# sakehl/SKA-SDP-Accelerate-gridding

Hardware: AMD Instinct MI355X
Metric: Mvis/s gridded (w-proj, 4096^2 grid) (higher is better)
Workload: dtype f64

## Files before the change

ska-sdp-accelerate-gridding_amd/csrc/api.hip:

```cpp

#include "common.h"
#include "imaging.h"

using namespace gridhip;

namespace {

int check_common(gridhip_ctx *ctx, int64_t H, int64_t Wd, const void *grid, int64_t n, const void *u,
                 const void *v, int64_t uv_stride)
{
    if (!ctx) return GRIDHIP_EINVAL;
    if (H <= 0 || Wd <= 0 || n < 0 || uv_stride < 1)
        return fail(ctx, GRIDHIP_EINVAL, "bad size (H=%lld Wd=%lld n=%lld uv_stride=%lld)", (long long)H,
                    (long long)Wd, (long long)n, (long long)uv_stride);
    if (!grid || (n > 0 && (!u || !v))) return fail(ctx, GRIDHIP_EINVAL, "null pointer");
    if (n > (int64_t)0x7fffff00) return fail(ctx, GRIDHIP_EUNSUPPORTED, "n must be < 2^31 per call");
    return GRIDHIP_OK;
}

int check_errors(gridhip_ctx *ctx)
{
    int32_t e = 0;
    GH_CHECK_HIP(ctx, hipMemcpyAsync(&e, ctx->d_scalars + 2, sizeof e, hipMemcpyDeviceToHost, ctx->stream));
    GH_CHECK_HIP(ctx, hipStreamSynchronize(ctx->stream));
// ... 22 lines not shown

static bool choose_parts(int64_t gh, int64_t gw, int side, int *py, int *px, int *sub)
{
    const int y = (int)((gh + side - 1) / side), x = (int)((gw + side - 1) / side);
    const int sy = (int)((gh + y - 1) / y), sx = (int)((gw + x - 1) / x);
    int sb = sy > sx ? sy : sx;
    if (sb < 5) sb = 5;
    if (y * x > 64) return false;
    *py = y;
    *px = x;
    *sub = sb;
    return true;
}

static void sorted_block(gridhip_ctx *ctx, Prep *p)
{
    if (ctx->opt.block != 0) return;
    const size_t per_cu = (size_t)ctx->max_lds / p->lds_sorted;
    p->block = per_cu >= 4 ? 256 : per_cu >= 2 ? 512 : 1024;
}

int prepare(gridhip_ctx *ctx, int64_t H, int64_t Wd, int64_t W, int64_t Q, int64_t gh, int64_t gw, int64_t n, Prep *p)
{
    *p = Prep();
    p->nrec = n;
    int rc = make_geom(ctx, H, Wd, W, Q, gh, gw, n, &p->g, &p->block, &p->lds);
    if (rc == GRIDHIP_OK) {
        const bool want = ctx->opt.sort == 1 || (ctx->opt.sort == 0 && n / (int64_t)p->g.nbins >= 256);
        const bool old_parts = ctx->opt.subfoot == 1 && gh > 16;
        p->sorted = want && !old_parts && sorted_plan(ctx, p->g, p->block, &p->nkeys, &p->batch, &p->lds_sorted);
        if (p->sorted) {
            p->g.chunk = p->batch;
            sorted_block(ctx, p);
        }
        if (p->sorted || ctx->opt.sort == 2) return GRIDHIP_OK;
    } else if (rc != GRIDHIP_EUNSUPPORTED || ctx->opt.tile != 0)
        return rc;
    int py, px, sub;
    const int side = ctx->opt.subfoot == 1 ? 16 : 32;
    if (ctx->opt.sort != 2 && (gh != gw || gh > side || gh < 5) && choose_parts(gh, gw, side, &py, &px, &sub) &&
        n * (int64_t)(py * px) < (int64_t)0x7fffff00 && W * Q * Q * (int64_t)(py * px) < ((int64_t)1 << 30)) {
        Prep q;
        const int P = py * px;
        q.nrec = n * P;
        if (make_geom(ctx, H, Wd, W, Q, sub, sub, q.nrec, &q.g, &q.block, &q.lds, P) == GRIDHIP_OK) {
            q.g.fgh = (int32_t)gh;
            q.g.fgw = (int32_t)gw;
            q.g.py = py;
            q.g.px = px;
            q.g.P = P;
            q.g.nvis = (int32_t)(n > 0 ? n : 1);
            q.g.nslices = (int32_t)(W * Q * Q * P);
            set_rec_bits(&q.g);
            set_div_magic(&q.g);
            const bool want = ctx->opt.sort == 1 || (ctx->opt.sort == 0 && q.nrec / (int64_t)q.g.nbins >= 256);
            q.sorted = want && sorted_plan(ctx, q.g, q.block, &q.nkeys, &q.batch, &q.lds_sorted);
            if (q.sorted) {
                q.g.chunk = q.batch;
                sorted_block(ctx, &q);
                *p = q;
                return GRIDHIP_OK;
            }
        }
    }
    if (rc == GRIDHIP_EUNSUPPORTED) {
        p->direct = true;
        return GRIDHIP_OK;
    }
    return rc;
}

int tile_kernels(gridhip_ctx *ctx, const Prep &p, const double *gcf, const double **out)
{
    ctx->last_path = p.direct ? 4 : !p.sorted ? 3 : p.g.P > 1 || p.g.fgh != p.g.gh || p.g.fgw != p.g.gw ? 2 : 1;
    ctx->last_geom[0] = p.g.ngroups;
    ctx->last_geom[1] = p.g.Tx;
    ctx->last_geom[2] = p.g.Ty;
    ctx->last_geom[3] = p.g.imoff > 0;
    *out = gcf;
    if (p.g.P == 1 && p.g.fgh == p.g.gh && p.g.fgw == p.g.gw) return GRIDHIP_OK;
    const int64_t nsl = (int64_t)p.g.W * p.g.Q * p.g.Q;
    const size_t elems = (size_t)nsl * p.g.P * p.g.gh * p.g.gw;
    GH_CHECK(ws_reserve(ctx, ctx->ktab, elems * 16));
    int blocks = (int)((elems + 255) / 256);
    if (blocks > ctx->num_cu * 16) blocks = ctx->num_cu * 16;
    hipLaunchKernelGGL(pad_kernels_kernel, dim3(blocks), dim3(256), 0, ctx->stream, p.g, nsl, (const double2 *)gcf,
                       (double2 *)ctx->ktab.ptr);
    GH_CHECK_HIP(ctx, hipGetLastError());
    *out = (const double *)ctx->ktab.ptr;
    return GRIDHIP_OK;
}

int upload_inputs(gridhip_ctx *ctx, GridInputs &d, size_t cells, const double *grid, int64_t n, int64_t uv_stride,
                  const double *u, const double *v, const double *vis, const int64_t *wbin, const double *gcf,
                  size_t gcf_elems)
{
    if (grid) {
        GH_CHECK(d.grid.upload(ctx, grid, cells * 16));
    } else {
        GH_CHECK(d.grid.alloc(ctx, cells * 16));
        GH_CHECK_HIP(ctx, hipMemsetAsync(d.grid.p, 0, cells * 16, ctx->stream));
    }
    const size_t span = n > 0 ? (size_t)(n - 1) * uv_stride + 1 : 0;
    GH_CHECK(d.u.upload(ctx, u, span * 8));
    GH_CHECK(d.v.upload(ctx, v, span * 8));
    GH_CHECK(vis ? d.vis.upload(ctx, vis, (size_t)n * 16) : d.vis.alloc(ctx, (size_t)n * 16));
    if (wbin) GH_CHECK(d.wbin.upload(ctx, wbin, (size_t)n * 8));
    if (gcf) GH_CHECK(d.gcf.upload(ctx, gcf, gcf_elems * 16));
    return GRIDHIP_OK;
}

// ... 179 lines not shown
```

ska-sdp-accelerate-gridding_amd/csrc/common.h:

```cpp
#pragma once
#include <hip/hip_runtime.h>
#include <stdint.h>
#include <stdio.h>
#include <string>
#include <unordered_set>

#include "../../include/gridhip.h"

namespace gridhip {

struct VisRec {
    int32_t lxy;
    int32_t kslice;
    int32_t orig;
};
typedef unsigned long long RecWord;

struct Geom {
    int64_t H, Wd;
    int32_t W, Q, gh, gw;
    int32_t Tx, Ty;
    int32_t offx, offy;
    int32_t ntx, nty;
    int32_t ntiles;
    int32_t ngroups;
    int32_t nbins;
    int32_t ldw;
    int32_t lrows, lcols;
    int32_t chunk;
    int32_t dbg;
    int32_t per_vis;
    int32_t nrec;
    int32_t nvis;
    int32_t nslices;
    int32_t fgh, fgw, px, py, P;
    int32_t ob, kb;
    int32_t dense;
    int32_t npersist;
    int32_t budget;
    int32_t imoff;
    uint32_t mTx, mTy, mW, mP, mPx;
    int32_t sTx, sTy, sW, sP, sPx;
};

static inline void div_magic(int64_t d, uint32_t *m, int32_t *s)
{
    if (d <= 1) {
        *m = 0;
        *s = -1;
        return;
    }
    int l = 0;
    while (((int64_t)1 << l) < d) ++l;
    const unsigned __int128 num = (unsigned __int128)1 << (31 + l);
    *m = (uint32_t)((num + (unsigned __int128)d - 1) / (unsigned __int128)d);
    *s = l - 1;
}
__device__ __forceinline__ uint32_t udiv_magic(uint32_t x, uint32_t m, int32_t s)
{
    return s < 0 ? x : __umulhi(x, m) >> s;
}
static inline void set_div_magic(Geom *g)
{
    div_magic(g->Tx, &g->mTx, &g->sTx);
    div_magic(g->Ty, &g->mTy, &g->sTy);
    div_magic(g->W, &g->mW, &g->sW);
    div_magic(g->P, &g->mP, &g->sP);
    div_magic(g->px, &g->mPx, &g->sPx);
}

static inline int bits_for(int64_t count)
{
    int b = 1;
    while (((int64_t)1 << b) < count) ++b;
    return b;
}
// ... 182 lines not shown
```

ska-sdp-accelerate-gridding_amd/csrc/ctx.hip:

```cpp
#include <stdarg.h>
#include <string.h>

#include <stdlib.h>

#include "common.h"
#include "imaging.h"

namespace gridhip {

int fail(gridhip_ctx *ctx, int code, const char *fmt, ...)
{
    char buf[512];
    va_list ap;
    va_start(ap, fmt);
    vsnprintf(buf, sizeof buf, fmt, ap);
    va_end(ap);
    if (ctx) ctx->err = buf;
    return code;
}

int ws_reserve(gridhip_ctx *ctx, Workspace &ws, size_t bytes)
{
    if (bytes <= ws.bytes) return GRIDHIP_OK;
    GH_CHECK_HIP(ctx, hipDeviceSynchronize());
// ... 52 lines not shown
    return l;
}

static int lds_pitch(int lcols, int gw)
{
    int p = lcols;
    while (p % 32 != gw % 32) ++p;
    return p;
}

size_t tables_bytes(const Geom &g)
{
    size_t ints = (size_t)g.nbins + ((size_t)g.nbins + 1) +
                  (size_t)g.ngroups * ((size_t)g.ntiles + 1) + (size_t)g.nbins;
    return ints * sizeof(int32_t);
}

Tables tables_of(gridhip_ctx *ctx, const Geom &g)
{
    Tables t;
    int32_t *p = (int32_t *)ctx->tables.ptr;
    t.bin_count = p;
    p += g.nbins;
    t.bin_start = p;
    p += g.nbins + 1;
    t.work_start = p;
    p += (size_t)g.ngroups * (g.ntiles + 1);
    t.cursor = p;
    t.scalars = ctx->d_scalars;
    return t;
}

static int make_geom1(gridhip_ctx *ctx, int64_t H, int64_t Wd, int64_t W, int64_t Q, int64_t gh, int64_t gw, int64_t n,
                      Geom *g, int *block, size_t *lds_bytes, int parts);

int make_geom(gridhip_ctx *ctx, int64_t H, int64_t Wd, int64_t W, int64_t Q, int64_t gh,
              int64_t gw, int64_t n, Geom *g, int *block, size_t *lds_bytes, int parts)
{
    GH_CHECK(make_geom1(ctx, H, Wd, W, Q, gh, gw, n, g, block, lds_bytes, parts));
    if (g->imoff > 0) {
        const int64_t planes = (W + g->ngroups - 1) / g->ngroups + 1;
        const size_t hist = (size_t)((planes * Q * Q * parts + 1 + 3) & ~(int64_t)3) * 4;
        if (2 * (size_t)g->imoff + hist + 128 > (size_t)ctx->max_lds) GH_CHECK(make_geom1(ctx, H, Wd, W, Q, gh, gw, n, g, block, lds_bytes, 0));
    }
    return GRIDHIP_OK;
}

static int make_geom1(gridhip_ctx *ctx, int64_t H, int64_t Wd, int64_t W, int64_t Q, int64_t gh, int64_t gw, int64_t n,
                      Geom *g, int *block, size_t *lds_bytes, int parts)
{
    if (H <= 0 || Wd <= 0 || W <= 0 || Q <= 0 || gh <= 0 || gw <= 0)
        return fail(ctx, GRIDHIP_EINVAL, "non-positive dimension");
    if (H > (1 << 30) || Wd > (1 << 30) || W * Q * Q > (1LL << 30) || gh > 1024 || gw > 1024)
        return fail(ctx, GRIDHIP_EUNSUPPORTED, "shape outside tile-kernel limits");
    memset(g, 0, sizeof *g);
    g->H = H;
    g->Wd = Wd;
    g->W = (int32_t)W;
    g->Q = (int32_t)Q;
    g->gh = (int32_t)gh;
    g->gw = (int32_t)gw;
    g->nvis = (int32_t)(n > 0 ? n : 1);
    g->nrec = g->nvis;
    g->nslices = (int32_t)(W * Q * Q);
    g->fgh = (int32_t)gh;
    g->fgw = (int32_t)gw;
    g->px = g->py = g->P = 1;
    g->per_vis = 0;
    set_rec_bits(g);
    if (ctx->opt.rec_bits >= 100 && ctx->opt.rec_bits <= 164 && g->ob + g->kb + 14 < ctx->opt.rec_bits - 100)
        g->kb = (int32_t)(ctx->opt.rec_bits - 100) - 14 - g->ob;

    const size_t lds_cap = (size_t)ctx->max_lds - 1024;
    const bool bt_ok = parts > 0 && ctx->opt.bigtile != 2 && ctx->opt.tile == 0 && ctx->opt.tile_x == 0 && gh == gw && gh >= 5 && gh <= 32;
    auto plane_for = [&](int tx, int ty) {
        return (size_t)lds_pitch(tx + (int)gw - 1, (int)gw) * (size_t)(ty + (int)gh - 1) * 8;
    };
    auto tiles_of = [&](int tx, int ty) {
        const int ox = (((int)gw - 1 + tx - 1) / tx) * tx, oy = (((int)gh - 1 + ty - 1) / ty) * ty;
        return (int64_t)((Wd - 1 + ox) / tx + 1) * (int64_t)((H - 1 + oy) / ty + 1);
    };
    auto auto_groups = [&](int64_t ntiles) {
        const double work = (double)n / (double)ntiles * ((double)gh * (double)gw / 225.0);
        return W < 8 ? 1 : work >= 8000.0 ? 8 : work >= 1200.0 ? 4 : work >= 600.0 ? 2 : 1;
    };
    int64_t ng_est = ctx->opt.wgroups ? ctx->opt.wgroups : (W >= 8 ? 8 : 1);
    auto largest_tile = [&](bool big, int *otx, int *oty) {
        const size_t hist_need = (size_t)(((W + ng_est - 1) / ng_est + 2) * Q * Q * (parts > 0 ? parts : 1)) * 4 + 1024;
        const size_t hist_room = big ? hist_need : (hist_need > 24576 && hist_need < 65536 * 4 ? hist_need : 24576);
        const size_t plane_cap = big ? lds_cap : 65528;
        size_t best = 0;
        if (hist_room + 8192 > lds_cap) return best;
        for (int tx = 8; tx <= 128; ++tx) {
            const int pitch = lds_pitch(tx + (int)gw - 1, (int)gw);
            if (tx < 128 && lds_pitch(tx + 1 + (int)gw - 1, (int)gw) == pitch) continue;
            int rows = (int)(plane_cap / ((size_t)pitch * 8));
            if ((size_t)rows * pitch * 16 > lds_cap - hist_room) rows = (int)((lds_cap - hist_room) / ((size_t)pitch * 16));
            int ty = rows - ((int)gh - 1);
            if (ty > 128) ty = 128;
            if (ty < 8) continue;
            if ((size_t)tx * ty > best) {
                best = (size_t)tx * ty;
                *otx = tx;
                *oty = ty;
            }
        }
        return best;
    };
    bool bigtile = false;
    int Tx = (int)ctx->opt.tile_x, Ty = (int)ctx->opt.tile_y;
    if (ctx->opt.tile) Tx = Ty = (int)ctx->opt.tile;
    if ((Tx == 0) != (Ty == 0)) return fail(ctx, GRIDHIP_EINVAL, "tile_x and tile_y go together");
    if (Tx == 0) {
        size_t best = largest_tile(false, &Tx, &Ty);
        if (best > 0 && bt_ok) {
            const int64_t tiles = ((H + Ty - 1) / Ty) * ((Wd + Tx - 1) / Tx);
            const bool sparse = n >= ((int64_t)1 << 22) && n < 2 * tiles * W * Q * Q;
            int bx = 0, by = 0;
            if (!ctx->opt.wgroups) ng_est = auto_groups(tiles_of(Tx, Ty));
            if ((ctx->opt.bigtile == 1 || sparse) && largest_tile(true, &bx, &by) > best) {
                best = (size_t)bx * by;
                Tx = bx;
                Ty = by;
                bigtile = true;
            }
        }
        if (best == 0) {
            Tx = Ty = 8;
            if (plane_for(8, 8) * 2 > lds_cap)
                return fail(ctx, GRIDHIP_EUNSUPPORTED, "a %lldx%lld kernel does not fit an LDS tile", (long long)gh, (long long)gw);
        }
        while ((Tx > 16 || Ty > 16) && ((H + Ty - 1) / Ty) * ((Wd + Tx - 1) / Tx) < 1024) {
            if (Ty >= Tx)
                --Ty;
            else
                --Tx;
        }
    }
    if (Tx < 8 || Tx > 128 || Ty < 8 || Ty > 128) return fail(ctx, GRIDHIP_EINVAL, "tile sides must be in 8..128");
    if (plane_for(Tx, Ty) * 2 > lds_cap)
        return fail(ctx, GRIDHIP_EUNSUPPORTED, "tile %dx%d with %lldx%lld kernel needs %zu B of LDS", Tx, Ty,
                    (long long)gh, (long long)gw, plane_for(Tx, Ty) * 2);
    g->Tx = Tx;
    g->Ty = Ty;
    g->imoff = bigtile && plane_for(Tx, Ty) > 65528 ? (int32_t)plane_for(Tx, Ty) : 0;
    g->lcols = Tx + (int)gw - 1;
    g->lrows = Ty + (int)gh - 1;
    g->ldw = lds_pitch(g->lcols, (int)gw);
    g->offx = (((int)gw - 1 + Tx - 1) / Tx) * Tx;
    g->offy = (((int)gh - 1 + Ty - 1) / Ty) * Ty;
    g->ntx = (int)((Wd - 1 + g->offx) / Tx) + 1;
    g->nty = (int)((H - 1 + g->offy) / Ty) + 1;
    if ((int64_t)g->ntx * g->nty > (1 << 24)) return fail(ctx, GRIDHIP_EUNSUPPORTED, "too many tiles");
    g->ntiles = g->ntx * g->nty;

    int ng = (int)ctx->opt.wgroups;
    if (ng == 0) {
        ng = auto_groups(g->ntiles);
        const int64_t cap = ((int64_t)ctx->max_lds - 8192) / 4;
        if (ng == 8 && (int64_t)g->ntiles * 8 > 4 * cap) ng = 4;
    }
    if (ng > W) ng = (int)W;
    if (W * ng >= ((int64_t)1 << 31)) ng = 1;
    if (ng < 1 || ng > 16) return fail(ctx, GRIDHIP_EINVAL, "wgroups must be in 1..16");
    g->ngroups = ng;
    g->nbins = ng * g->ntiles;
    set_div_magic(g);
    g->dense = ctx->opt.wtable ? (ctx->opt.wtable >= 3 ? 2 : ctx->opt.wtable == 2 ? 1 : 0)
                               : (gh >= 15 && n >= 2 * (int64_t)g->ntiles * W * Q * Q) ? 1 : (g->imoff > 0 && gh == 15) ? 2 : 0;

    int chunk = (int)ctx->opt.chunk;
    if (chunk == 0) chunk = 8192;
    if (chunk < 64) chunk = 64;
    g->chunk = chunk;
    g->dbg = (int32_t)ctx->opt.dbg;

    *lds_bytes = plane_for(Tx, Ty) * 2;
    int b = (int)ctx->opt.block;
    if (b == 0) {
        size_t per_cu = (size_t)ctx->max_lds / *lds_bytes;
        b = per_cu >= 4 ? 256 : per_cu >= 2 ? 512 : 1024;
    }
    if (b < 64 || b > 1024 || (b & 63)) return fail(ctx, GRIDHIP_EINVAL, "block must be a multiple of 64 in 64..1024");
    *block = b;
    (void)n;
    return GRIDHIP_OK;
}

}

using namespace gridhip;

extern "C" {

int gridhip_version(void) { return GRIDHIP_VERSION; }

const char *gridhip_strerror(int code)
{
    switch (code) {
        case GRIDHIP_OK: return "ok";
        case GRIDHIP_EINVAL: return "invalid argument";
        case GRIDHIP_ENOMEM: return "out of memory";
// ... 326 lines not shown
```

ska-sdp-accelerate-gridding_amd/csrc/tile_sorted.hip:

```cpp
#include "tile_common.h"

namespace gridhip {

__device__ __forceinline__ double readlane_f64(double x, int l)
{
    return __hiloint2double(__builtin_amdgcn_readlane(__double2hiint(x), l),
                            __builtin_amdgcn_readlane(__double2loint(x), l));
}

constexpr int SORTED_IM_OFF = 65528;

__device__ const int cut15[3][16] = {{0, 106, 211, 317, 422, 500, 578, 655, 733, 781, 829, 877, 926, 958, 991, 1024},
                                     {0, 108, 221, 329, 434, 513, 596, 677, 754, 800, 852, 898, 943, 969, 998, 1024},
                                     {0, 100, 202, 303, 401, 480, 562, 641, 718, 769, 824, 875, 925, 957, 992, 1024}};

struct SortedItem {
    int32_t valid, tile, grp, staged;
};

template <int S, bool DEGRID, int ABL = 0, bool AW = false, bool BT = false>
__global__ void __launch_bounds__(1024, 4) tile_grid_sorted_kernel(Geom g, const RecWord *__restrict__ recs,
                                                                const int32_t *__restrict__ bin_start,
                                                                const int32_t *__restrict__ work_start,
                                                                const double2 *__restrict__ gcf,
                                                                double2 *__restrict__ vis,
                                                                double *__restrict__ grid, int nkeys, int batch,
                                                                int32_t *__restrict__ scalars,
                                                                double2 *__restrict__ sorted_vals,
                                                                uint2 *__restrict__ sorted_mo)
{
    extern __shared__ double lds[];
    constexpr int S2 = S * S;
    constexpr int TAIL0 = S2 - ((S2 + 63) / 64 - 1) * 64;
    constexpr int EXTRA = DEGRID ? 0 : (TAIL0 > 32 && TAIL0 <= 34) ? TAIL0 - 32 : (S2 > 256 && TAIL0 <= 2) ? TAIL0 : 0;
    constexpr int S2E = S2 - EXTRA;
    constexpr int NSTEP_ALL = (S2E + 63) / 64;
    constexpr int TAIL = S2E - (NSTEP_ALL - 1) * 64;
    constexpr int MAXST = DEGRID ? 4 : 5;
    constexpr int FP = (NSTEP_ALL + MAXST - 1) / MAXST;
    constexpr int KST = (NSTEP_ALL + FP - 1) / FP;
    constexpr int REM = NSTEP_ALL % FP;
    constexpr int PBASE = NSTEP_ALL / FP;
    constexpr int NSTEP = KST;
    constexpr int LASTS = (REM == 0 ? KST : KST - 1) - 1;
    constexpr bool PAIR = !DEGRID && TAIL == 32;
    const int tid = threadIdx.x, nthr = blockDim.x;
    const int lane = tid & 63, wave = __builtin_amdgcn_readfirstlane(tid >> 6), nw = nthr >> 6;
    const int plane = g.lrows * g.ldw;
    const int IMO = BT ? g.imoff / 8 : SORTED_IM_OFF / 8;
    double *lre = lds, *lim = lds + IMO;
    int32_t *hist = reinterpret_cast<int32_t *>(lim + plane);
    const int hist_words = (nkeys + 1 + 3) & ~3;
    SortedItem *desc = reinterpret_cast<SortedItem *>(hist + hist_words);
    double2 *svals_wg = sorted_vals + (size_t)blockIdx.x * 2 * batch;
    uint2 *smo_wg = sorted_mo + (size_t)blockIdx.x * 2 * batch;
    int32_t *sorig_wg = reinterpret_cast<int32_t *>(sorted_vals) + (size_t)blockIdx.x * 2 * batch;

    constexpr bool STAGE_VALS = !DEGRID && AW;
    constexpr bool STAGE_ORIG = DEGRID && AW;
    const bool solo = nw == 1;
    const bool is_sorter = wave == nw - 1;
    if (is_sorter && !solo && !(g.dbg & 512)) __builtin_amdgcn_s_setprio(3);
    const bool is_walker = solo || !is_sorter;
    const int nwalk = solo ? 1 : nw - 1;
    const int ncell = g.lrows * g.lcols;

    if (blockIdx.x == 0 && tid == 0) {
        long long *st = reinterpret_cast<long long *>(scalars + 20);
        st[0] = (long long)__builtin_amdgcn_s_memtime();
        st[1] = (long long)__builtin_amdgcn_s_memrealtime();
    }
    long long prof[7] = {0, 0, 0, 0, 0, 0, 0}, pt = 0;
#define GH_STAMP(i_)                        \
    if ((ABL & 16) && lane == 0) {          \
        const long long now_ = clock64();   \
        prof[i_] += now_ - pt;              \
        pt = now_;                          \
    }
    if ((ABL & 16) && lane == 0) pt = clock64();

    int32_t *queue = scalars + 4;
    int turn = 0;
    int items_left = ((int)blockIdx.x >= g.npersist) ? g.budget : 0x7fffffff;
    auto prepare = [&](int slot) {
// ... 57 lines not shown
            }
            int base = incl - sum;
            for (int i = lo; i < hi; ++i) {
                const int c = hist[i];
                hist[i] = base;
                base += c;
            }
        }
        __builtin_amdgcn_fence(__ATOMIC_ACQ_REL, "wavefront");
        __builtin_amdgcn_wave_barrier();
        GH_STAMP(2)
        int bad = 0;
        for (int r0 = lane; r0 < cnt; r0 += 8 * 64) {
            VisRec rec[8];
            double2 val[8];
            bool off[8];
#pragma unroll
            for (int q = 0; q < 8; ++q) rec[q] = load_rec(recs, b_lo + min(r0 + q * 64, cnt - 1), g, &off[q]);
            if (STAGE_VALS) {
#pragma unroll
                for (int q = 0; q < 8; ++q) val[q] = (ABL & 8) ? make_double2(1.0, (double)q) : load_nt(vis + rec[q].orig);
            }
#pragma unroll
            for (int q = 0; q < 8; ++q) {
                if (r0 + q * 64 >= cnt) break;
                int key = rec[q].kslice - first_slice;
                if (AW) key = (int)((unsigned)key % (unsigned)nkeys);
                if (off[q] || (unsigned)key >= (unsigned)nkeys) {
                    ++bad;
                    continue;
                }
                const int pos = atomicAdd(&hist[key], 1);
                if ((unsigned)pos < (unsigned)batch) {
                    smo[pos] = make_uint2(((uint32_t)key << 16) | (uint32_t)((rec[q].lxy >> 16) * g.ldw + (rec[q].lxy & 0xffff)),
                                          (uint32_t)(AW ? rec[q].kslice : rec[q].orig));
                    if (STAGE_VALS) svals[pos] = val[q];
                    if (STAGE_ORIG) sorig[pos] = rec[q].orig;
                } else
                    ++bad;
            }
        }
        if (bad) atomicAdd(&scalars[2], bad);
        __builtin_amdgcn_fence(__ATOMIC_ACQ_REL, "wavefront");
        __builtin_amdgcn_wave_barrier();
        if (lane == 0) {
            SortedItem d;
            d.valid = 1;
            d.tile = w.tile;
            d.grp = grp;
            d.staged = hist[nkeys - 1];
            desc[slot] = d;
        }
        GH_STAMP(3)
    };

    int loff[NSTEP];
    const bool tail_ok = lane < TAIL || TAIL == 64;
#pragma unroll
    for (int s = 0; s < NSTEP; ++s) {
        int t = s * 64 + lane;
        if (FP == 1 && s == NSTEP - 1 && !tail_ok) t = PAIR ? s * 64 + lane - 32 : 0;
        loff[s] = (t / S) * g.ldw + (t % S);
    }
    const int ttail = tail_ok ? LASTS * 64 + lane : PAIR ? LASTS * 64 + lane - 32 : 0;
    const int lrow = lane / S, lcol = lane - lrow * S;

    auto walk = [&](int slot, int staged, int first_slice) {
        const double2 *svals = svals_wg + (size_t)slot * batch;
        const uint2 *smo = smo_wg + (size_t)slot * batch;
        const int32_t *sorig = sorig_wg + (size_t)slot * batch;
        int seg_lo, seg_hi;
        if (nwalk == 15 && !DEGRID && !(g.dbg & 256)) {
            seg_lo = (int)(((int64_t)staged * cut15[g.dense][wave]) >> 10);
            seg_hi = (int)(((int64_t)staged * cut15[g.dense][wave + 1]) >> 10);
        } else {
            seg_lo = (int)(((int64_t)staged * wave) / nwalk);
            seg_hi = (int)(((int64_t)staged * (wave + 1)) / nwalk);
        }
        if (seg_lo >= seg_hi) return;
        auto load_list = [&](int b0, uint2 &mo, double2 &v, int32_t &o) {
            const int idx = max(min(b0 + lane, seg_hi - 1), seg_lo);
            mo = smo[idx];
            if (STAGE_VALS) v = svals[idx];
            if (STAGE_ORIG) o = sorig[idx];
        };
        auto load_value = [&](const uint2 &mo, double2 &v) {
            if (!DEGRID && !STAGE_VALS) v = (ABL & 8) ? make_double2(1.0, 2.0) : load_nt(vis + mo.y);
        };
        auto part_step0 = [&](int part) { return FP == 1 ? 0 : part * PBASE + min(part, REM); };
        auto part_nst = [&](int part) { return (FP == 1 || REM == 0 || part < REM) ? KST : KST - 1; };
        auto issue = [&](double2(&k)[NSTEP], int key, int len, int part) {
            key = min(max(key, 0), (AW ? g.nslices : nkeys) - 1);
            asm volatile("" : "+s"(key));
            const double2 *kp = gcf + (size_t)(first_slice + key) * S2 + 64 * part_step0(part);
            if (ABL & 4) {
// ... 62 lines not shown
                    return;
                }
                start = (int)__builtin_ctzll(bits);
                bits &= bits - 1;
                len = (bits ? (int)__builtin_ctzll(bits) : bcnt) - start;
                key = lastKey = AW ? __builtin_amdgcn_readlane((int)mo.y, start)
                                   : (int)((uint32_t)__builtin_amdgcn_readlane((int)mo.x, start) >> 16);
                if (FP > 1) {
                    part = 0;
                    curKey = key;
                    curStart = start;
                    curLen = len;
                    curPart = 0;
                }
            };
            auto process = [&](const double2(&k)[NSTEP], int start, int len, int part) {
                int lo[NSTEP];
                const bool lastp = FP == 1 || part == FP - 1;
                const bool shortp = FP > 1 && part_nst(part) < KST;
                if (FP == 1) {
#pragma unroll
                    for (int s = 0; s < NSTEP; ++s) lo[s] = loff[s];
                } else {
                    const int st0 = part_step0(part);
#pragma unroll
                    for (int s = 0; s < NSTEP; ++s) {
                        const int tl = 64 * (st0 + s);
                        const int A = tl / S, B = tl - A * S;
                        int lr = lrow, lc = lcol;
                        if (PAIR && s == LASTS && lastp && lane >= 32) {
                            lr = (lane - 32) / S;
                            lc = (lane - 32) - lr * S;
                        }
                        const int carry = (B + lc >= S) ? g.ldw - S : 0;
                        lo[s] = (A + lr) * g.ldw + B + lc + carry;
                    }
                }
                if (!DEGRID) {
                    int i = 0;
                    if (PAIR && lastp) {
                        for (; i + 1 < len; i += 2) {
                            const int j0 = start + i, j1 = j0 + 1;
                            const int lb0 = (int)((uint32_t)__builtin_amdgcn_readlane((int)mo.x, j0) & 0xffff);
                            const int lb1 = (int)((uint32_t)__builtin_amdgcn_readlane((int)mo.x, j1) & 0xffff);
                            const double vx0 = readlane_f64(vB.x, j0), vy0 = readlane_f64(vB.y, j0);
                            const double vx1 = readlane_f64(vB.x, j1), vy1 = readlane_f64(vB.y, j1);
#pragma unroll
                            for (int s = 0; s < LASTS; ++s) {
                                double *cell = lre + (lb0 + lo[s]);
                                if (ABL & 1) continue;
                                __hip_atomic_fetch_add(cell, vx0 * k[s].x - vy0 * k[s].y, __ATOMIC_RELAXED,
                                                       __HIP_MEMORY_SCOPE_WORKGROUP);
                                __hip_atomic_fetch_add(cell + IMO, vx0 * k[s].y + vy0 * k[s].x,
                                                       __ATOMIC_RELAXED, __HIP_MEMORY_SCOPE_WORKGROUP);
                            }
#pragma unroll
                            for (int s = 0; s < LASTS; ++s) {
                                double *cell = lre + (lb1 + lo[s]);
                                if (ABL & 1) continue;
                                __hip_atomic_fetch_add(cell, vx1 * k[s].x - vy1 * k[s].y, __ATOMIC_RELAXED,
                                                       __HIP_MEMORY_SCOPE_WORKGROUP);
                                __hip_atomic_fetch_add(cell + IMO, vx1 * k[s].y + vy1 * k[s].x,
                                                       __ATOMIC_RELAXED, __HIP_MEMORY_SCOPE_WORKGROUP);
                            }
                            const double2 kl = k[LASTS];
                            double re, im;
                            int a;
                            if (lane < 32) {
// ... 91 lines not shown
            constexpr int NSETS = 3;
            double2 kS[NSETS][NSTEP];
            int keyS[NSETS], startS[NSETS], lenS[NSETS], partS[NSETS] = {0, 0, 0};
            static_assert(NSETS == 3, "initialiser of partS");
#pragma unroll
            for (int r = 0; r < NSETS - 1; ++r) {
                advance(keyS[r], startS[r], lenS[r], partS[r]);
                issue(kS[r], keyS[r], lenS[r], partS[r]);
            }
            int done = 0;
            for (;;) {
#pragma unroll
                for (int r = 0; r < NSETS; ++r) {
                    const int nx = (r + NSETS - 1) % NSETS;
                    advance(keyS[nx], startS[nx], lenS[nx], partS[nx]);
                    issue(kS[nx], keyS[nx], lenS[nx], partS[nx]);
                    asm volatile("" ::: "memory");
                    __builtin_amdgcn_sched_barrier(0);
                    process(kS[r], startS[r], lenS[r], partS[r]);
                    __builtin_amdgcn_sched_barrier(0);
                    if (FP == 1 || partS[r] == FP - 1) done += lenS[r];
                }
                if (done >= bcnt) break;
            }
            if (done > bcnt) {
#pragma unroll
                for (int r = 0; r < NSETS - 1; ++r) asm volatile("" ::"v"(kS[r][0].x), "v"(kS[r][NSTEP - 1].y));
            }
            if (EXTRA > 0 && !(ABL & 1) && lane < bcnt) {
                const int lb = (int)(mo.x & 0xffff);
#pragma unroll
                for (int e = 0; e < EXTRA; ++e) {
                    const int t = S2 - EXTRA + e;
                    double *cell = lre + (lb + (t / S) * g.ldw + (t % S));
                    __hip_atomic_fetch_add(cell, vB.x * kx[e].x - vB.y * kx[e].y, __ATOMIC_RELAXED,
                                           __HIP_MEMORY_SCOPE_WORKGROUP);
                    __hip_atomic_fetch_add(cell + IMO, vB.x * kx[e].y + vB.y * kx[e].x, __ATOMIC_RELAXED,
                                           __HIP_MEMORY_SCOPE_WORKGROUP);
                }
            }
        }
    };

    const int fl_r0 = (tid >> 1) / g.lcols, fl_c0 = (tid >> 1) - fl_r0 * g.lcols;
    const int fl_dr = (nthr >> 1) / g.lcols, fl_dc = (nthr >> 1) - fl_dr * g.lcols;

    if (is_sorter) prepare(0);
    if (!DEGRID) {
        for (int i = tid; i < plane; i += nthr) {
            lre[i] = 0.0;
            lim[i] = 0.0;
        }
    }
    __syncthreads();
    for (int cur = 0;; cur ^= 1) {
        const SortedItem d = desc[cur];
        if (!d.valid) break;
        const int first_plane = (d.grp * g.W + g.ngroups - 1) / g.ngroups;
        const int first_slice = first_plane * g.Q * g.Q * g.P;
        const int tx = d.tile % g.ntx, ty = d.tile / g.ntx;
        const int64_t ox = (int64_t)tx * g.Tx - g.offx, oy = (int64_t)ty * g.Ty - g.offy;
        if (DEGRID) {
            const double2 *gsrc = reinterpret_cast<const double2 *>(grid);
            for (int c = tid; c < ncell; c += nthr) {
                const int r_ = c / g.lcols, c_ = c - r_ * g.lcols;
                const int64_t gx = ox + c_, gy = oy + r_;
                double2 v = make_double2(0.0, 0.0);
                if (gx >= 0 && gy >= 0 && gx < g.Wd && gy < g.H) v = gsrc[gy * g.Wd + gx];
                lre[r_ * g.ldw + c_] = v.x;
                lim[r_ * g.ldw + c_] = v.y;
            }
            __syncthreads();
        }
        const long long walk_t0 = (ABL & 16) ? clock64() : 0;
        if (is_sorter && !solo) prepare(cur ^ 1);
        if (is_walker) {
            if ((ABL & 16) && wave == 0 && lane == 0) pt = clock64();
            walk(cur, d.staged, first_slice);
            if ((ABL & 16) && wave == 0) GH_STAMP(4)
        }
        if (solo) prepare(cur ^ 1);
        if ((ABL & 16) && lane == 0)
            atomicAdd(reinterpret_cast<unsigned long long *>(scalars + 32) + 8 + wave, (unsigned long long)(clock64() - walk_t0));
        __syncthreads();
        if ((ABL & 16) && wave == 0) GH_STAMP(5)
        if (DEGRID) continue;

        {
            const int comp = tid & 1;
            int r_ = fl_r0, c_ = fl_c0;
            for (int e = tid; e < 2 * ncell; e += nthr) {
                const int64_t gx = ox + c_, gy = oy + r_;
                double *cell = (comp ? lim : lre) + r_ * g.ldw + c_;
                c_ += fl_dc;
                r_ += fl_dr;
                if (c_ >= g.lcols) {
                    c_ -= g.lcols;
                    ++r_;
                }
                const double val = *cell;
                if (val == 0.0) continue;
                *cell = 0.0;
                if ((ABL & 2) || gx < 0 || gy < 0 || gx >= g.Wd || gy >= g.H) continue;
                unsafeAtomicAdd(grid + 2 * (gy * g.Wd + gx) + comp, val);
            }
        }
        __syncthreads();
        if ((ABL & 16) && wave == 0) GH_STAMP(6)
    }
    if (blockIdx.x == 0 && tid == 0) {
        long long *st = reinterpret_cast<long long *>(scalars + 20);
        st[2] = (long long)__builtin_amdgcn_s_memtime();
        st[3] = (long long)__builtin_amdgcn_s_memrealtime();
    }
    if ((ABL & 16) && lane == 0 && (wave == 0 || (is_sorter && !solo))) {
        unsigned long long *out = reinterpret_cast<unsigned long long *>(scalars + 32);
        for (int i = 0; i < 7; ++i)
            if (prof[i]) atomicAdd(&out[i], (unsigned long long)prof[i]);
    }
#undef GH_STAMP
}

bool sorted_plan(const gridhip_ctx *ctx, const Geom &g, int block, int *nkeys, int *batch, size_t *lds_bytes)
{
    if (g.gh != g.gw || g.gh < 5 || g.gh > (g.per_vis ? 16 : 32)) return false;
    const int planes = (g.W + g.ngroups - 1) / g.ngroups + 1;
    const int64_t keys = g.per_vis ? 4096 : (int64_t)planes * g.Q * g.Q * g.P;
    if (keys >= 65536) return false;
    const size_t plane = (size_t)g.lrows * g.ldw * 8;
    if (plane > (size_t)(g.imoff > 0 ? g.imoff : SORTED_IM_OFF)) return false;
    const size_t tile = (size_t)(g.imoff > 0 ? g.imoff : SORTED_IM_OFF) + plane;
    const size_t hist = (size_t)((keys + 1 + 3) & ~3) * 4;
    if (tile + hist + 128 > (size_t)ctx->max_lds) return false;
    (void)block;
    int c = ctx->opt.chunk ? (int)ctx->opt.chunk : 16384;
    c = c < 64 ? 64 : c > 16384 ? 16384 : c;
    *nkeys = (int)keys;
    *batch = c;
    *lds_bytes = tile + hist + 128;
    return true;
}

int launch_tile_grid_sorted(gridhip_ctx *ctx, const Geom &g_in, int block, size_t lds_bytes, int nkeys, int batch,
                            int64_t n, const double *gcf, const double *vis, double *grid, bool degrid)
{
    Geom g = g_in;
    Tables t = tables_of(ctx, g);
    const RecWord *recs = (const RecWord *)ctx->recs.ptr;
    if (g.chunk > batch) return fail(ctx, GRIDHIP_EINVAL, "sorted kernel: chunk %d exceeds its work-item capacity %d", g.chunk, batch);
    if (g.per_vis && g.imoff > 0) return fail(ctx, GRIDHIP_EUNSUPPORTED, "no big-tile form of the aw tile kernel");
    int per_cu = (int)((size_t)ctx->max_lds / lds_bytes);
    per_cu = per_cu < 1 ? 1 : per_cu > 4 ? 4 : per_cu;
    if (per_cu * block > 2048) per_cu = 2048 / block > 0 ? 2048 / block : 1;
    int cus = ctx->num_cu - (int)ctx->opt.reserve_cus;
    if (cus < g.ngroups) cus = g.ngroups;
    int nblk = cus * per_cu;
    nblk = ctx->opt.reserve_cus ? (nblk / g.ngroups) * g.ngroups : ((nblk + g.ngroups - 1) / g.ngroups) * g.ngroups;
    const int most = work_blocks(g, n);
    if (nblk > most) nblk = most > g.ngroups ? (most / g.ngroups) * g.ngroups : g.ngroups;
    g.npersist = nblk;
    g.budget = 0;
    if (ctx->opt.yield_cus > 0 && !ctx->opt.reserve_cus) {
        int k = (((int)ctx->opt.yield_cus + 31) / 32) * 32 * per_cu;
        k = (k / g.ngroups) * g.ngroups;
        if (k > 0 && nblk - k >= g.ngroups) {
            g.npersist = nblk - k;
            g.budget = 8;
            int extra = most - g.npersist;
            extra = extra > 2048 ? 2048 : extra;
            extra = (extra / g.ngroups) * g.ngroups;
            nblk = g.npersist + (extra > k ? extra : k);
        }
    }
    const dim3 gr(nblk), bl(block);
    const size_t nlist = (size_t)nblk * 2 * batch, nvals = g.per_vis ? nlist : 0;
    GH_CHECK(ws_reserve(ctx, ctx->sorted, nvals * 16 + nlist * 8));
    double2 *svals = (double2 *)ctx->sorted.ptr;
    uint2 *smo = (uint2 *)(svals + nvals);
    launch_clear(ctx, t.scalars + 4, 16, (g.dbg & 16) ? t.scalars + 32 : nullptr, (g.dbg & 16) ? 64 : 0);
#define GH_LAUNCH_(S_, D_, B_)                                                                                   \
    do {                                                                                                         \
        GH_CHECK(raise_lds(ctx, tile_grid_sorted_kernel<S_, D_, 0, false, B_>));                                 \
        hipLaunchKernelGGL((tile_grid_sorted_kernel<S_, D_, 0, false, B_>), gr, bl, lds_bytes, ctx->stream, g, recs, \
                           t.bin_start, t.work_start, (const double2 *)gcf, (double2 *)vis, grid, nkeys, batch, \
                           t.scalars, svals, smo);                                                               \
    } while (0)
#define GH_LAUNCH(S_, D_)                \
    do {                                 \
        if (g.imoff > 0)                 \
            GH_LAUNCH_(S_, D_, true);    \
        else                             \
            GH_LAUNCH_(S_, D_, false);   \
    } while (0)
#define GH_LAUNCH_AW_(S_, D_)                                                                                    \
    do {                                                                                                         \
        GH_CHECK(raise_lds(ctx, tile_grid_sorted_kernel<S_, D_, 0, true>));                                      \
        hipLaunchKernelGGL((tile_grid_sorted_kernel<S_, D_, 0, true>), gr, bl, lds_bytes, ctx->stream, g, recs,  \
                           t.bin_start, t.work_start, (const double2 *)gcf, (double2 *)vis, grid, nkeys, batch, \
                           t.scalars, svals, smo);                                                               \
    } while (0)
#define GH_LAUNCH_AW(S_)                 \
    do {                                 \
        if (degrid)                      \
            GH_LAUNCH_AW_(S_, true);     \
        else                             \
            GH_LAUNCH_AW_(S_, false);    \
    } while (0)
#define GH_CASE(S_)             \
    case S_:                    \
        if (g.per_vis)          \
            GH_LAUNCH_AW(S_);   \
        else if (degrid)        \
            GH_LAUNCH(S_, true); \
        else                    \
            GH_LAUNCH(S_, false); \
        break;
#define GH_BIG(S_)                                                                  \
    case S_:                                                                        \
        if (g.per_vis) return fail(ctx, GRIDHIP_EUNSUPPORTED, "aw tile kernel: support %d", g.gh); \
        if (degrid)                                                                 \
            GH_LAUNCH(S_, true);                                                    \
        else                                                                        \
            GH_LAUNCH(S_, false);                                                   \
        break;
#define GH_ABL_BT(A_)                                                                                            \
    if (g.gh == 15 && !degrid && g.imoff > 0 && g.dbg == A_) {                                                   \
        GH_CHECK(raise_lds(ctx, tile_grid_sorted_kernel<15, false, A_, false, true>));                           \
        hipLaunchKernelGGL((tile_grid_sorted_kernel<15, false, A_, false, true>), gr, bl, lds_bytes, ctx->stream, g, recs, \
                           t.bin_start, t.work_start, (const double2 *)gcf, (double2 *)vis, grid, nkeys, batch, \
                           t.scalars, svals, smo);                                                               \
        GH_CHECK_HIP(ctx, hipGetLastError());                                                                    \
        return GRIDHIP_OK;                                                                                       \
    }
#define GH_ABL(A_)                                                                                               \
    if (g.gh == 15 && !degrid && g.imoff == 0 && g.dbg == A_) {                                                  \
        GH_CHECK(raise_lds(ctx, tile_grid_sorted_kernel<15, false, A_>));                                        \
        hipLaunchKernelGGL((tile_grid_sorted_kernel<15, false, A_>), gr, bl, lds_bytes, ctx->stream, g, recs,    \
                           t.bin_start, t.work_start, (const double2 *)gcf, (double2 *)vis, grid, nkeys, batch, \
                           t.scalars, svals, smo);                                                               \
        GH_CHECK_HIP(ctx, hipGetLastError());                                                                    \
        return GRIDHIP_OK;                                                                                       \
    }
#ifdef GRIDHIP_TUNING
    GH_ABL(1) GH_ABL(2) GH_ABL(3) GH_ABL(4) GH_ABL(5) GH_ABL(7) GH_ABL(8) GH_ABL(15) GH_ABL(16) GH_ABL_BT(16)
#endif
#undef GH_ABL
#undef GH_ABL_BT
    switch (g.gh) {
        GH_CASE(5) GH_CASE(6) GH_CASE(7) GH_CASE(8) GH_CASE(9) GH_CASE(10) GH_CASE(11) GH_CASE(12) GH_CASE(13)
        GH_CASE(14) GH_CASE(15) GH_CASE(16)
        GH_BIG(17) GH_BIG(18) GH_BIG(19) GH_BIG(20) GH_BIG(21) GH_BIG(22) GH_BIG(23) GH_BIG(24) GH_BIG(25) GH_BIG(26)
        GH_BIG(27) GH_BIG(28) GH_BIG(29) GH_BIG(30) GH_BIG(31) GH_BIG(32)
        default: return fail(ctx, GRIDHIP_EUNSUPPORTED, "no sorted instantiation for support %d", g.gh);
    }
#undef GH_CASE
#undef GH_BIG
#undef GH_LAUNCH
#undef GH_LAUNCH_
#undef GH_LAUNCH_AW
#undef GH_LAUNCH_AW_
    GH_CHECK_HIP(ctx, hipGetLastError());
    return GRIDHIP_OK;
}

}
```

Before: 9171.

## Interleave real/imag LDS planes with a compile-time offset and tuned row pitch

Replaces the sorted tile kernel's split real/imag LDS layout, which used a fixed 64 KB imaginary-plane offset or a runtime big-tile offset, with a per-support compile-time distance between real and imaginary cells inside a shared row of pitch R. The row pitch is chosen to keep bank alignment and to maximise the tile area that fits in LDS. This is meant to fit larger tiles into LDS without a separate BT template variant and to make the imaginary offset a constant, which reduces halo overhead and address arithmetic. It adds new geometry constraints and fallbacks when the layout does not fit, and it changes how tiles are sized on the non-big path.

```diff
diff --git a/ska-sdp-accelerate-gridding_amd/csrc/api.hip b/ska-sdp-accelerate-gridding_amd/csrc/api.hip
--- a/ska-sdp-accelerate-gridding_amd/csrc/api.hip
+++ b/ska-sdp-accelerate-gridding_amd/csrc/api.hip
@@ -78,6 +78,10 @@
         if (p->sorted) {
             p->g.chunk = p->batch;
             sorted_block(ctx, p);
+        }
+        if (!p->sorted && p->g.big) {
+            rc = make_geom(ctx, H, Wd, W, Q, gh, gw, n, &p->g, &p->block, &p->lds, -1);
+            if (rc != GRIDHIP_OK) return rc;
         }
         if (p->sorted || ctx->opt.sort == 2) return GRIDHIP_OK;
     } else if (rc != GRIDHIP_EUNSUPPORTED || ctx->opt.tile != 0)
@@ -122,7 +126,7 @@
     ctx->last_geom[0] = p.g.ngroups;
     ctx->last_geom[1] = p.g.Tx;
     ctx->last_geom[2] = p.g.Ty;
-    ctx->last_geom[3] = p.g.imoff > 0;
+    ctx->last_geom[3] = p.g.big;
     *out = gcf;
     if (p.g.P == 1 && p.g.fgh == p.g.gh && p.g.fgw == p.g.gw) return GRIDHIP_OK;
     const int64_t nsl = (int64_t)p.g.W * p.g.Q * p.g.Q;
diff --git a/ska-sdp-accelerate-gridding_amd/csrc/common.h b/ska-sdp-accelerate-gridding_amd/csrc/common.h
--- a/ska-sdp-accelerate-gridding_amd/csrc/common.h
+++ b/ska-sdp-accelerate-gridding_amd/csrc/common.h
@@ -38,10 +38,34 @@
     int32_t dense;
     int32_t npersist;
     int32_t budget;
-    int32_t imoff;
+    int32_t sR, sD, big;
     uint32_t mTx, mTy, mW, mP, mPx;
     int32_t sTx, sTy, sW, sP, sPx;
 };
+
+constexpr int SORTED_LDS_CELLS = (160 * 1024 - 1024 - 5632) / 8;
+constexpr int sorted_pitch(int cols, int S)
+{
+    int p = cols;
+    while (p % 32 != S % 32) ++p;
+    return p;
+}
+constexpr int sorted_im_dist(int S)
+{
+    int best = 0, dist = 0;
+    for (int pass = 0; pass < 2; ++pass)
+        for (int R = sorted_pitch(2 * (8 + S - 1), S); R <= 2 * (128 + S - 1) + 32; R += 32) {
+            int lcols = R / 2;
+            if (lcols > 128 + S - 1) lcols = 128 + S - 1;
+            int ty = SORTED_LDS_CELLS / R - (S - 1);
+            if (ty > 128) ty = 128;
+            if (ty < 8) continue;
+            const int cells = (lcols - (S - 1)) * ty;
+            if (pass == 0 && cells > best) best = cells;
+            if (pass == 1 && dist == 0 && cells * 100 >= best * 99) dist = R - lcols;
+        }
+    return dist;
+}
 
 static inline void div_magic(int64_t d, uint32_t *m, int32_t *s)
 {
diff --git a/ska-sdp-accelerate-gridding_amd/csrc/ctx.hip b/ska-sdp-accelerate-gridding_amd/csrc/ctx.hip
--- a/ska-sdp-accelerate-gridding_amd/csrc/ctx.hip
+++ b/ska-sdp-accelerate-gridding_amd/csrc/ctx.hip
@@ -108,22 +108,22 @@
 }
 
 static int make_geom1(gridhip_ctx *ctx, int64_t H, int64_t Wd, int64_t W, int64_t Q, int64_t gh, int64_t gw, int64_t n,
-                      Geom *g, int *block, size_t *lds_bytes, int parts);
+                      Geom *g, int *block, size_t *lds_bytes, int parts, bool allow_big);
 
 int make_geom(gridhip_ctx *ctx, int64_t H, int64_t Wd, int64_t W, int64_t Q, int64_t gh,
               int64_t gw, int64_t n, Geom *g, int *block, size_t *lds_bytes, int parts)
 {
-    GH_CHECK(make_geom1(ctx, H, Wd, W, Q, gh, gw, n, g, block, lds_bytes, parts));
-    if (g->imoff > 0) {
+    GH_CHECK(make_geom1(ctx, H, Wd, W, Q, gh, gw, n, g, block, lds_bytes, parts, true));
+    if (g->big) {
         const int64_t planes = (W + g->ngroups - 1) / g->ngroups + 1;
         const size_t hist = (size_t)((planes * Q * Q * parts + 1 + 3) & ~(int64_t)3) * 4;
-        if (2 * (size_t)g->imoff + hist + 128 > (size_t)ctx->max_lds) GH_CHECK(make_geom1(ctx, H, Wd, W, Q, gh, gw, n, g, block, lds_bytes, 0));
+        if ((size_t)g->sR * g->lrows * 8 + hist + 128 > (size_t)ctx->max_lds) GH_CHECK(make_geom1(ctx, H, Wd, W, Q, gh, gw, n, g, block, lds_bytes, parts, false));
     }
     return GRIDHIP_OK;
 }
 
 static int make_geom1(gridhip_ctx *ctx, int64_t H, int64_t Wd, int64_t W, int64_t Q, int64_t gh, int64_t gw, int64_t n,
-                      Geom *g, int *block, size_t *lds_bytes, int parts)
+                      Geom *g, int *block, size_t *lds_bytes, int parts, bool allow_big)
 {
     if (H <= 0 || Wd <= 0 || W <= 0 || Q <= 0 || gh <= 0 || gw <= 0)
         return fail(ctx, GRIDHIP_EINVAL, "non-positive dimension");
@@ -148,7 +148,7 @@
         g->kb = (int32_t)(ctx->opt.rec_bits - 100) - 14 - g->ob;
 
     const size_t lds_cap = (size_t)ctx->max_lds - 1024;
-    const bool bt_ok = parts > 0 && ctx->opt.bigtile != 2 && ctx->opt.tile == 0 && ctx->opt.tile_x == 0 && gh == gw && gh >= 5 && gh <= 32;
+    const bool bt_ok = allow_big && parts > 0 && ctx->opt.bigtile != 2 && ctx->opt.tile == 0 && ctx->opt.tile_x == 0 && gh == gw && gh >= 5 && gh <= 32;
     auto plane_for = [&](int tx, int ty) {
         return (size_t)lds_pitch(tx + (int)gw - 1, (int)gw) * (size_t)(ty + (int)gh - 1) * 8;
     };
@@ -161,17 +161,36 @@
         return W < 8 ? 1 : work >= 8000.0 ? 8 : work >= 1200.0 ? 4 : work >= 600.0 ? 2 : 1;
     };
     int64_t ng_est = ctx->opt.wgroups ? ctx->opt.wgroups : (W >= 8 ? 8 : 1);
+    const int sD = gh == gw && gh >= 5 && gh <= 32 ? sorted_im_dist((int)gh) : 0;
+    auto sorted_row = [&](int lcols) { return sD > 0 && lcols <= sD ? sorted_pitch(sD + lcols, (int)gw) : 0; };
     auto largest_tile = [&](bool big, int *otx, int *oty) {
         const size_t hist_need = (size_t)(((W + ng_est - 1) / ng_est + 2) * Q * Q * (parts > 0 ? parts : 1)) * 4 + 1024;
         const size_t hist_room = big ? hist_need : (hist_need > 24576 && hist_need < 65536 * 4 ? hist_need : 24576);
-        const size_t plane_cap = big ? lds_cap : 65528;
         size_t best = 0;
         if (hist_room + 8192 > lds_cap) return best;
+        if (big) {
+            for (int R = sorted_pitch(sD + 8 + (int)gw - 1, (int)gw); R <= 2 * sD + 31; R += 32) {
+                int tx = (R - sD < sD ? R - sD : sD) - ((int)gw - 1);
+                if (tx > 128) tx = 128;
+                int ty = (int)((lds_cap - hist_need) / ((size_t)R * 8)) - ((int)gh - 1);
+                if (ty > 128) ty = 128;
+                if (tx < 8 || ty < 8) continue;
+                if ((size_t)tx * ty > best) {
+                    best = (size_t)tx * ty;
+                    *otx = tx;
+                    *oty = ty;
+                }
+            }
+            return best;
+        }
         for (int tx = 8; tx <= 128; ++tx) {
             const int pitch = lds_pitch(tx + (int)gw - 1, (int)gw);
             if (tx < 128 && lds_pitch(tx + 1 + (int)gw - 1, (int)gw) == pitch) continue;
-            int rows = (int)(plane_cap / ((size_t)pitch * 8));
+            int rows = (int)(65528 / ((size_t)pitch * 8));
             if ((size_t)rows * pitch * 16 > lds_cap - hist_room) rows = (int)((lds_cap - hist_room) / ((size_t)pitch * 16));
+            const size_t sorted_hist = parts == 0 ? 4100 * 4 + 1024 : hist_need;
+            const int sr = parts < 0 ? 0 : sorted_row(tx + (int)gw - 1);
+            if (sr > 0 && (size_t)rows * sr * 8 > lds_cap - sorted_hist) rows = (int)((lds_cap - sorted_hist) / ((size_t)sr * 8));
             int ty = rows - ((int)gh - 1);
             if (ty > 128) ty = 128;
             if (ty < 8) continue;
@@ -214,15 +233,17 @@
         }
     }
     if (Tx < 8 || Tx > 128 || Ty < 8 || Ty > 128) return fail(ctx, GRIDHIP_EINVAL, "tile sides must be in 8..128");
-    if (plane_for(Tx, Ty) * 2 > lds_cap)
+    if (!bigtile && plane_for(Tx, Ty) * 2 > lds_cap)
         return fail(ctx, GRIDHIP_EUNSUPPORTED, "tile %dx%d with %lldx%lld kernel needs %zu B of LDS", Tx, Ty,
                     (long long)gh, (long long)gw, plane_for(Tx, Ty) * 2);
     g->Tx = Tx;
     g->Ty = Ty;
-    g->imoff = bigtile && plane_for(Tx, Ty) > 65528 ? (int32_t)plane_for(Tx, Ty) : 0;
+    g->big = bigtile;
     g->lcols = Tx + (int)gw - 1;
     g->lrows = Ty + (int)gh - 1;
     g->ldw = lds_pitch(g->lcols, (int)gw);
+    g->sD = sD;
+    g->sR = parts < 0 ? 0 : sorted_row(g->lcols);
     g->offx = (((int)gw - 1 + Tx - 1) / Tx) * Tx;
     g->offy = (((int)gh - 1 + Ty - 1) / Ty) * Ty;
     g->ntx = (int)((Wd - 1 + g->offx) / Tx) + 1;
@@ -243,7 +264,7 @@
     g->nbins = ng * g->ntiles;
     set_div_magic(g);
     g->dense = ctx->opt.wtable ? (ctx->opt.wtable >= 3 ? 2 : ctx->opt.wtable == 2 ? 1 : 0)
-                               : (gh >= 15 && n >= 2 * (int64_t)g->ntiles * W * Q * Q) ? 1 : (g->imoff > 0 && gh == 15) ? 2 : 0;
+                               : (gh >= 15 && n >= 2 * (int64_t)g->ntiles * W * Q * Q) ? 1 : (g->big && gh == 15) ? 2 : 0;
 
     int chunk = (int)ctx->opt.chunk;
     if (chunk == 0) chunk = 8192;
diff --git a/ska-sdp-accelerate-gridding_amd/csrc/tile_sorted.hip b/ska-sdp-accelerate-gridding_amd/csrc/tile_sorted.hip
--- a/ska-sdp-accelerate-gridding_amd/csrc/tile_sorted.hip
+++ b/ska-sdp-accelerate-gridding_amd/csrc/tile_sorted.hip
@@ -8,8 +8,6 @@
                             __builtin_amdgcn_readlane(__double2loint(x), l));
 }
 
-constexpr int SORTED_IM_OFF = 65528;
-
 __device__ const int cut15[3][16] = {{0, 106, 211, 317, 422, 500, 578, 655, 733, 781, 829, 877, 926, 958, 991, 1024},
                                      {0, 108, 221, 329, 434, 513, 596, 677, 754, 800, 852, 898, 943, 969, 998, 1024},
                                      {0, 100, 202, 303, 401, 480, 562, 641, 718, 769, 824, 875, 925, 957, 992, 1024}};
@@ -18,7 +16,7 @@
     int32_t valid, tile, grp, staged;
 };
 
-template <int S, bool DEGRID, int ABL = 0, bool AW = false, bool BT = false>
+template <int S, bool DEGRID, int ABL = 0, bool AW = false>
 __global__ void __launch_bounds__(1024, 4) tile_grid_sorted_kernel(Geom g, const RecWord *__restrict__ recs,
                                                                 const int32_t *__restrict__ bin_start,
                                                                 const int32_t *__restrict__ work_start,
@@ -46,10 +44,11 @@
     constexpr bool PAIR = !DEGRID && TAIL == 32;
     const int tid = threadIdx.x, nthr = blockDim.x;
     const int lane = tid & 63, wave = __builtin_amdgcn_readfirstlane(tid >> 6), nw = nthr >> 6;
-    const int plane = g.lrows * g.ldw;
-    const int IMO = BT ? g.imoff / 8 : SORTED_IM_OFF / 8;
+    const int R = g.sR;
+    constexpr int IMO = sorted_im_dist(S);
+    const int tile_cells = g.lrows * R;
     double *lre = lds, *lim = lds + IMO;
-    int32_t *hist = reinterpret_cast<int32_t *>(lim + plane);
+    int32_t *hist = reinterpret_cast<int32_t *>(lds + tile_cells);
     const int hist_words = (nkeys + 1 + 3) & ~3;
     SortedItem *desc = reinterpret_cast<SortedItem *>(hist + hist_words);
     double2 *svals_wg = sorted_vals + (size_t)blockIdx.x * 2 * batch;
@@ -173,7 +172,7 @@
                 }
                 const int pos = atomicAdd(&hist[key], 1);
                 if ((unsigned)pos < (unsigned)batch) {
-                    smo[pos] = make_uint2(((uint32_t)key << 16) | (uint32_t)((rec[q].lxy >> 16) * g.ldw + (rec[q].lxy & 0xffff)),
+                    smo[pos] = make_uint2(((uint32_t)key << 16) | (uint32_t)((rec[q].lxy >> 16) * R + (rec[q].lxy & 0xffff)),
                                           (uint32_t)(AW ? rec[q].kslice : rec[q].orig));
                     if (STAGE_VALS) svals[pos] = val[q];
                     if (STAGE_ORIG) sorig[pos] = rec[q].orig;
@@ -201,7 +200,7 @@
     for (int s = 0; s < NSTEP; ++s) {
         int t = s * 64 + lane;
         if (FP == 1 && s == NSTEP - 1 && !tail_ok) t = PAIR ? s * 64 + lane - 32 : 0;
-        loff[s] = (t / S) * g.ldw + (t % S);
+        loff[s] = (t / S) * R + (t % S);
     }
     const int ttail = tail_ok ? LASTS * 64 + lane : PAIR ? LASTS * 64 + lane - 32 : 0;
     const int lrow = lane / S, lcol = lane - lrow * S;
@@ -330,8 +329,8 @@
                             lr = (lane - 32) / S;
                             lc = (lane - 32) - lr * S;
                         }
-                        const int carry = (B + lc >= S) ? g.ldw - S : 0;
-                        lo[s] = (A + lr) * g.ldw + B + lc + carry;
+                        const int carry = (B + lc >= S) ? R - S : 0;
+                        lo[s] = (A + lr) * R + B + lc + carry;
                     }
                 }
                 if (!DEGRID) {
@@ -489,7 +488,7 @@
 #pragma unroll
                 for (int e = 0; e < EXTRA; ++e) {
                     const int t = S2 - EXTRA + e;
-                    double *cell = lre + (lb + (t / S) * g.ldw + (t % S));
+                    double *cell = lre + (lb + (t / S) * R + (t % S));
                     __hip_atomic_fetch_add(cell, vB.x * kx[e].x - vB.y * kx[e].y, __ATOMIC_RELAXED,
                                            __HIP_MEMORY_SCOPE_WORKGROUP);
                     __hip_atomic_fetch_add(cell + IMO, vB.x * kx[e].y + vB.y * kx[e].x, __ATOMIC_RELAXED,
@@ -504,10 +503,7 @@
 
     if (is_sorter) prepare(0);
     if (!DEGRID) {
-        for (int i = tid; i < plane; i += nthr) {
-            lre[i] = 0.0;
-            lim[i] = 0.0;
-        }
+        for (int i = tid; i < tile_cells; i += nthr) lds[i] = 0.0;
     }
     __syncthreads();
     for (int cur = 0;; cur ^= 1) {
@@ -524,8 +520,8 @@
                 const int64_t gx = ox + c_, gy = oy + r_;
                 double2 v = make_double2(0.0, 0.0);
                 if (gx >= 0 && gy >= 0 && gx < g.Wd && gy < g.H) v = gsrc[gy * g.Wd + gx];
-                lre[r_ * g.ldw + c_] = v.x;
-                lim[r_ * g.ldw + c_] = v.y;
+                lre[r_ * R + c_] = v.x;
+                lim[r_ * R + c_] = v.y;
             }
             __syncthreads();
         }
@@ -548,7 +544,7 @@
             int r_ = fl_r0, c_ = fl_c0;
             for (int e = tid; e < 2 * ncell; e += nthr) {
                 const int64_t gx = ox + c_, gy = oy + r_;
-                double *cell = (comp ? lim : lre) + r_ * g.ldw + c_;
+                double *cell = (comp ? lim : lre) + r_ * R + c_;
                 c_ += fl_dc;
                 r_ += fl_dr;
                 if (c_ >= g.lcols) {
@@ -584,9 +580,9 @@
     const int planes = (g.W + g.ngroups - 1) / g.ngroups + 1;
     const int64_t keys = g.per_vis ? 4096 : (int64_t)planes * g.Q * g.Q * g.P;
     if (keys >= 65536) return false;
-    const size_t plane = (size_t)g.lrows * g.ldw * 8;
-    if (plane > (size_t)(g.imoff > 0 ? g.imoff : SORTED_IM_OFF)) return false;
-    const size_t tile = (size_t)(g.imoff > 0 ? g.imoff : SORTED_IM_OFF) + plane;
+    if (g.sR <= 0 || g.sD != sorted_im_dist(g.gh) || g.lcols > g.sD || g.sD + g.lcols > g.sR || g.sR % 32 != g.gw % 32) return false;
+    if ((int64_t)(g.lrows - g.gh) * g.sR + (g.lcols - g.gw) > 65535) return false;
+    const size_t tile = (size_t)g.sR * g.lrows * 8;
     const size_t hist = (size_t)((keys + 1 + 3) & ~3) * 4;
     if (tile + hist + 128 > (size_t)ctx->max_lds) return false;
     (void)block;
@@ -605,7 +601,6 @@
     Tables t = tables_of(ctx, g);
     const RecWord *recs = (const RecWord *)ctx->recs.ptr;
     if (g.chunk > batch) return fail(ctx, GRIDHIP_EINVAL, "sorted kernel: chunk %d exceeds its work-item capacity %d", g.chunk, batch);
-    if (g.per_vis && g.imoff > 0) return fail(ctx, GRIDHIP_EUNSUPPORTED, "no big-tile form of the aw tile kernel");
     int per_cu = (int)((size_t)ctx->max_lds / lds_bytes);
     per_cu = per_cu < 1 ? 1 : per_cu > 4 ? 4 : per_cu;
     if (per_cu * block > 2048) per_cu = 2048 / block > 0 ? 2048 / block : 1;
@@ -635,19 +630,12 @@
     double2 *svals = (double2 *)ctx->sorted.ptr;
     uint2 *smo = (uint2 *)(svals + nvals);
     launch_clear(ctx, t.scalars + 4, 16, (g.dbg & 16) ? t.scalars + 32 : nullptr, (g.dbg & 16) ? 64 : 0);
-#define GH_LAUNCH_(S_, D_, B_)                                                                                   \
+#define GH_LAUNCH(S_, D_)                                                                                        \
     do {                                                                                                         \
-        GH_CHECK(raise_lds(ctx, tile_grid_sorted_kernel<S_, D_, 0, false, B_>));                                 \
-        hipLaunchKernelGGL((tile_grid_sorted_kernel<S_, D_, 0, false, B_>), gr, bl, lds_bytes, ctx->stream, g, recs, \
+        GH_CHECK(raise_lds(ctx, tile_grid_sorted_kernel<S_, D_>));                                               \
+        hipLaunchKernelGGL((tile_grid_sorted_kernel<S_, D_>), gr, bl, lds_bytes, ctx->stream, g, recs,           \
                            t.bin_start, t.work_start, (const double2 *)gcf, (double2 *)vis, grid, nkeys, batch, \
                            t.scalars, svals, smo);                                                               \
-    } while (0)
-#define GH_LAUNCH(S_, D_)                \
-    do {                                 \
-        if (g.imoff > 0)                 \
-            GH_LAUNCH_(S_, D_, true);    \
-        else                             \
-            GH_LAUNCH_(S_, D_, false);   \
     } while (0)
 #define GH_LAUNCH_AW_(S_, D_)                                                                                    \
     do {                                                                                                         \
@@ -680,17 +668,8 @@
         else                                                                        \
             GH_LAUNCH(S_, false);                                                   \
         break;
-#define GH_ABL_BT(A_)                                                                                            \
-    if (g.gh == 15 && !degrid && g.imoff > 0 && g.dbg == A_) {                                                   \
-        GH_CHECK(raise_lds(ctx, tile_grid_sorted_kernel<15, false, A_, false, true>));                           \
-        hipLaunchKernelGGL((tile_grid_sorted_kernel<15, false, A_, false, true>), gr, bl, lds_bytes, ctx->stream, g, recs, \
-                           t.bin_start, t.work_start, (const double2 *)gcf, (double2 *)vis, grid, nkeys, batch, \
-                           t.scalars, svals, smo);                                                               \
-        GH_CHECK_HIP(ctx, hipGetLastError());                                                                    \
-        return GRIDHIP_OK;                                                                                       \
-    }
 #define GH_ABL(A_)                                                                                               \
-    if (g.gh == 15 && !degrid && g.imoff == 0 && g.dbg == A_) {                                                  \
+    if (g.gh == 15 && !degrid && g.dbg == A_) {                                                                  \
         GH_CHECK(raise_lds(ctx, tile_grid_sorted_kernel<15, false, A_>));                                        \
         hipLaunchKernelGGL((tile_grid_sorted_kernel<15, false, A_>), gr, bl, lds_bytes, ctx->stream, g, recs,    \
                            t.bin_start, t.work_start, (const double2 *)gcf, (double2 *)vis, grid, nkeys, batch, \
@@ -699,10 +678,9 @@
         return GRIDHIP_OK;                                                                                       \
     }
 #ifdef GRIDHIP_TUNING
-    GH_ABL(1) GH_ABL(2) GH_ABL(3) GH_ABL(4) GH_ABL(5) GH_ABL(7) GH_ABL(8) GH_ABL(15) GH_ABL(16) GH_ABL_BT(16)
+    GH_ABL(1) GH_ABL(2) GH_ABL(3) GH_ABL(4) GH_ABL(5) GH_ABL(7) GH_ABL(8) GH_ABL(15) GH_ABL(16)
 #endif
 #undef GH_ABL
-#undef GH_ABL_BT
     switch (g.gh) {
         GH_CASE(5) GH_CASE(6) GH_CASE(7) GH_CASE(8) GH_CASE(9) GH_CASE(10) GH_CASE(11) GH_CASE(12) GH_CASE(13)
         GH_CASE(14) GH_CASE(15) GH_CASE(16)
@@ -713,7 +691,6 @@
 #undef GH_CASE
 #undef GH_BIG
 #undef GH_LAUNCH
-#undef GH_LAUNCH_
 #undef GH_LAUNCH_AW
 #undef GH_LAUNCH_AW_
     GH_CHECK_HIP(ctx, hipGetLastError());
```

After: 9168, median of 2. Within noise of the previous version (-0.0%).
